# intel/pailliercryptolib

Hardware: AMD Instinct MI355X
Metric: 2048-bit modexps/sec (encrypt+decrypt) (higher is better)
Workload: dtype u64

## Files before the change

### pailliercryptolib_amd/csrc/hensel_ps_bal.hpp

```cpp
#ifndef PAILLIERCRYPTOLIB_AMD_CSRC_HENSEL_PS_BAL_HPP_
#define PAILLIERCRYPTOLIB_AMD_CSRC_HENSEL_PS_BAL_HPP_

#include "hensel_ps.hpp"

#ifndef PGPU_PSB_DOUBLED
#define PGPU_PSB_DOUBLED 1
#endif
#ifndef PGPU_PSB_KARATSUBA
#define PGPU_PSB_KARATSUBA 1
#endif

namespace pgpu {

template <int LB>
__device__ __forceinline__ int32_t psb_sext(uint32_t v) { return __builtin_amdgcn_sbfe((int)v, 0u, (unsigned)LB); }

__device__ __forceinline__ void psb_mac(int64_t& acc, int32_t x, int32_t y) { acc += (int64_t)x * y; }
__device__ __forceinline__ void psb_mac_pinned(int64_t& acc, int32_t x, int32_t y) {
  acc += (int64_t)x * y;
  asm volatile("" ::"v"(acc));
}

__device__ __forceinline__ void psb_mac_wrap(int64_t& acc, int32_t x, int32_t y) {
  acc = (int64_t)((uint64_t)acc + (uint64_t)((int64_t)x * y));
}

template <int K, int LB>
struct PsbFits {
  static constexpr bool value = 2 * (LB - 1) < 62 && LB + 6 < 62 &&
                                3 * (uint64_t)K * ((uint64_t)1 << (2 * (LB - 1))) + ((uint64_t)1 << (LB + 6)) < ((uint64_t)1 << 63);
};

template <int K, int LB, int NP, bool SYM, int QMODE, bool DBL = false, bool KARA = false>
__device__ __forceinline__ void psb_montmul(int32_t (&r)[K], const int32_t (&x1)[K], const int32_t (&y1)[K],
                                            const int32_t (&x2)[K], const int32_t (&y2)[K], const int32_t (&n)[K],
                                            uint32_t n0inv, int32_t (&qio)[K]) {
  static_assert(!(SYM && NP != 1), "a symmetric product is a single one");
  static_assert(SYM || !DBL, "the doubled operand belongs to the symmetric product");
  static_assert(!KARA || (NP == 1 && !SYM && K % 2 == 0), "the split serves the single product of two operands, in two halves");
  static_assert(PsbFits<K, LB>::value, "a column sums up to 3K products below 2^(2(LB-1)): must stay below 2^63");
  constexpr int H = K / 2;
  int32_t q[K];
  int64_t acc = 0;
  int32_t onev = 1;
  asm("" : "+v"(onev));
  int32_t dx[KARA ? H : 1], dy[KARA ? H : 1];
  uint64_t lo[KARA ? 2 * H - 1 : 1], hi[KARA ? 2 * H - 1 : 1];
  if constexpr (KARA) {
#pragma unroll
    for (int j = 0; j < H; ++j) {
      dx[j] = x1[j] - x1[H + j];
      dy[j] = y1[H + j] - y1[j];
    }
  }
  ps_static_for<2 * K>([&](auto colc) __attribute__((always_inline)) {
    constexpr int col = decltype(colc)::value;
    {
      constexpr int ilo = col < K ? 0 : col - K + 1;
      constexpr int ihi = col < K ? col : K;
      if constexpr (ihi > ilo) {
        ps_static_for<ihi - ilo>([&](auto ic) __attribute__((always_inline)) {
          constexpr int i = ilo + decltype(ic)::value;
          if constexpr (PGPU_PS_PIN == 2 || (PGPU_PS_PIN == 1 && SYM)) psb_mac_pinned(acc, q[i], n[col - i]);
          else psb_mac(acc, q[i], n[col - i]);
        });
      }
    }
    if constexpr (SYM) {
      constexpr int ilo = col < K ? 0 : col - K + 1;
      constexpr int ihi = (col + 1) / 2;
      if constexpr (DBL) {
        if constexpr (ihi > ilo) {
          ps_static_for<ihi - ilo>([&](auto ic) __attribute__((always_inline)) {
            constexpr int i = ilo + decltype(ic)::value;
            psb_mac(acc, x1[i], y1[col - i]);
          });
        }
        if constexpr (col % 2 == 0) psb_mac(acc, y1[col / 2], y1[col / 2]);
      } else {
        if constexpr (ihi > ilo) {
          int64_t cross = 0;
          ps_static_for<ihi - ilo>([&](auto ic) __attribute__((always_inline)) {
            constexpr int i = ilo + decltype(ic)::value;
            psb_mac(cross, x1[i], x1[col - i]);
          });
          acc = (int64_t)((uint64_t)acc + ((uint64_t)cross << 1));
        }
        if constexpr (col % 2 == 0) psb_mac(acc, x1[col / 2], x1[col / 2]);
      }
    } else if constexpr (KARA) {
      if constexpr (col <= 2 * H - 2) {
        constexpr int ilo = col < H ? 0 : col - H + 1;
        constexpr int ihi = col < H ? col + 1 : H;
        int64_t s = 0;
        ps_static_for<ihi - ilo>([&](auto ic) __attribute__((always_inline)) {
          constexpr int i = ilo + decltype(ic)::value;
          psb_mac_wrap(s, x1[i], y1[col - i]);
        });
        lo[col] = (uint64_t)s;
        acc = (int64_t)((uint64_t)acc + lo[col]);
      }
      if constexpr (col >= H && col <= 3 * H - 2) {
        constexpr int k = col - H;
        constexpr int ilo = k < H ? 0 : k - H + 1;
        constexpr int ihi = k < H ? k + 1 : H;
        int64_t s = 0;
        ps_static_for<ihi - ilo>([&](auto ic) __attribute__((always_inline)) {
          constexpr int i = ilo + decltype(ic)::value;
          psb_mac_wrap(s, x1[H + i], y1[H + k - i]);
        });
        hi[k] = (uint64_t)s;
        acc = (int64_t)((uint64_t)acc + (lo[k] + hi[k]));
        ps_static_for<ihi - ilo>([&](auto ic) __attribute__((always_inline)) {
          constexpr int i = ilo + decltype(ic)::value;
          psb_mac_wrap(acc, dx[i], dy[k - i]);
        });
      }
      if constexpr (col >= 2 * H && col <= 4 * H - 2) acc = (int64_t)((uint64_t)acc + hi[col - 2 * H]);
    } else {
      constexpr int ilo = col < K ? 0 : col - K + 1;
      constexpr int ihi = col < K ? col + 1 : K;
      ps_static_for<ihi - ilo>([&](auto ic) __attribute__((always_inline)) {
        constexpr int i = ilo + decltype(ic)::value;
        if constexpr (PGPU_PS_PIN == 2) {
          psb_mac_pinned(acc, x1[i], y1[col - i]);
          if constexpr (NP == 2) psb_mac_pinned(acc, x2[i], y2[col - i]);
        } else {
          psb_mac(acc, x1[i], y1[col - i]);
          if constexpr (NP == 2) psb_mac(acc, x2[i], y2[col - i]);
        }
      });
    }
    if constexpr (col < K) {
      if constexpr (QMODE == 2) psb_mac(acc, qio[col], onev);
      q[col] = psb_sext<LB>((uint32_t)acc * n0inv);
      psb_mac(acc, q[col], n[0]);
      acc >>= LB;
      if constexpr (QMODE == 1) qio[col] = q[col];
    } else {
      r[col - K] = psb_sext<LB>((uint32_t)acc);
      if constexpr (col + 1 < 2 * K) acc = (acc + ((int64_t)1 << (LB - 1))) >> LB;
    }
  });
}

template <int K>
__device__ __forceinline__ uint32_t (&psb_bits(int32_t (&v)[K]))[K] { return reinterpret_cast<uint32_t(&)[K]>(v); }
template <int K>
__device__ __forceinline__ const uint32_t (&psb_bits(const int32_t (&v)[K]))[K] { return reinterpret_cast<const uint32_t(&)[K]>(v); }

template <int K, int LB, bool DBL = (PGPU_PSB_DOUBLED != 0), bool KARA = (PGPU_PSB_KARATSUBA != 0)>
__device__ __forceinline__ void psb_pairsqr(int32_t (&a)[K], int32_t (&b)[K], const int32_t (&n)[K], uint32_t n0inv) {
  int32_t qd[K], t[K];
  if constexpr (DBL) {
    int32_t a2[K];
#pragma unroll
    for (int j = 0; j < K; ++j) a2[j] = a[j] * 2;
    psb_montmul<K, LB, 1, true, 1, true>(t, a2, a, a2, a, n, n0inv, qd);
    psb_montmul<K, LB, 1, false, 2, false, KARA>(b, a2, b, a2, b, n, n0inv, qd);
  } else {
    psb_montmul<K, LB, 1, true, 1>(t, a, a, a, a, n, n0inv, qd);
#pragma unroll
    for (int j = 0; j < K; ++j) b[j] *= 2;
    psb_montmul<K, LB, 1, false, 2>(b, a, b, a, b, n, n0inv, qd);
  }
#pragma unroll
  for (int j = 0; j < K; ++j) a[j] = t[j];
}

template <int K, int LB, bool KARA = (PGPU_PSB_KARATSUBA != 0)>
__device__ __forceinline__ void psb_pairmul(int32_t (&a)[K], int32_t (&b)[K], const int32_t (&c)[K], const int32_t (&d)[K],
                                            const int32_t (&n)[K], uint32_t n0inv, uint4* slot) {
  int32_t qd[K];
  {
    int32_t t[K];
    ps_park_store<K>(slot, psb_bits<K>(b));
    __builtin_amdgcn_sched_barrier(0);
    psb_montmul<K, LB, 1, false, 1, false, KARA>(t, a, c, a, c, n, n0inv, qd);
    __builtin_amdgcn_sched_barrier(0);
    ps_park_swap<K>(slot, psb_bits<K>(b), psb_bits<K>(t));
    __builtin_amdgcn_sched_barrier(0);
  }
  psb_montmul<K, LB, 2, false, 2>(b, a, d, b, c, n, n0inv, qd);
  __builtin_amdgcn_sched_barrier(0);
  ps_park_load<K>(psb_bits<K>(a), slot);
}

template <int K, int LB>
__device__ __forceinline__ void psb_mul(int32_t (&r)[K], const int32_t (&x)[K], const int32_t (&y)[K], const int32_t (&n)[K],
                                        uint32_t n0inv) {
  int32_t none[K];
  psb_montmul<K, LB, 1, false, 0>(r, x, y, x, y, n, n0inv, none);
}

template <int K, int LB>
__device__ __forceinline__ void psb_add(int32_t (&a)[K], const int32_t (&k)[K]) {
  int32_t c = 0;
#pragma unroll
  for (int j = 0; j < K; ++j) {
    const int32_t u = a[j] + k[j] + c;
    a[j] = j + 1 < K ? psb_sext<LB>((uint32_t)u) : u;
    c = (u + (1 << (LB - 1))) >> LB;
  }
}

template <int K, int LB, int NI>
__device__ __forceinline__ void psb_relimb(int32_t (&out)[K], const uint32_t (&in)[NI]) {
  static_assert(NI <= K, "the chunk must fit");
  uint32_t c = 0;
#pragma unroll
  for (int j = 0; j < K; ++j) {
    const uint32_t u = (j < NI ? in[j] : 0u) + c;
    out[j] = j + 1 < K ? psb_sext<LB>(u) : (int32_t)u;
    c = (u + (1u << (LB - 1))) >> LB;
  }
}

template <int K, int LB>
__device__ __forceinline__ int32_t psb_canon(uint32_t (&out)[K], const int32_t (&v)[K]) {
  int32_t c = 0;
#pragma unroll
  for (int j = 0; j < K; ++j) {
    const int32_t u = v[j] + c;
    out[j] = (uint32_t)u & PsLimb<LB>::mask;
    c = u >> LB;
  }
  return c;
}

template <int K, int LB>
__device__ __forceinline__ void psb_entry_from_pair_row(const HenselArgs& A, int side, size_t elem, const int32_t (&n)[K],
                                                        uint32_t n0inv, uint4* slot, int32_t (&a)[K], int32_t (&b)[K],
                                                        int32_t (&ma)[K], int32_t (&mb)[K]) {
  static_assert(LB == kLimbBits, "the row limbs are re-balanced, not re-cut");
  constexpr int NI = (K * LB - 2) / LB + 1;
#define HCTX(field) (side ? A.ctx[1].field : A.ctx[0].field)
  const uint32_t* row = A.ct_pair + elem * A.ct_pair_stride;
  int32_t acc_a[K], acc_b[K];
#pragma unroll
  for (int j = 0; j < K; ++j) acc_a[j] = acc_b[j] = 0;
#pragma unroll 1
  for (int i = 0; i < A.pchunks; ++i) {
    const int first = i * A.pchunk_limbs;
    uint32_t za[NI], zb[NI];
    int32_t cb[K], tb[K];
#pragma unroll
    for (int j = 0; j < NI; ++j) {
      const bool in = j < A.pchunk_limbs && first + j < A.pair_l2;
      za[j] = in ? row[first + j] : 0u;
      zb[j] = in ? row[A.pair_l2 + first + j] : 0u;
    }
#pragma unroll
    for (int j = 0; j < K; ++j) {
      b[j] = 0;
      cb[j] = (int32_t)HCTX(pcb)[(size_t)i * K + j];
      ma[j] = (int32_t)HCTX(pconv)[(size_t)i * 2 * K + j];
      mb[j] = (int32_t)HCTX(pconv)[(size_t)i * 2 * K + K + j];
    }
    int32_t zl[K];
    psb_relimb<K, LB, NI>(zl, zb);
    psb_mul<K, LB>(tb, zl, cb, n, n0inv);
    psb_relimb<K, LB, NI>(a, za);
    psb_pairmul<K, LB, false>(a, b, ma, mb, n, n0inv, slot);
    psb_add<K, LB>(b, tb);
    psb_add<K, LB>(acc_a, a);
    psb_add<K, LB>(acc_b, b);
  }
#pragma unroll
  for (int j = 0; j < K; ++j) {
    a[j] = ma[j] = acc_a[j];
    b[j] = mb[j] = acc_b[j];
  }
#undef HCTX
}

template <int K, int LB>
__device__ __forceinline__ void psb_exit_words(const HenselArgs& A, int side, size_t elem, bool live, uint4* slot,
                                               const int32_t (&n)[K], uint32_t n0inv, int32_t (&a)[K], int32_t (&b)[K],
                                               int32_t (&ma)[K], int32_t (&mb)[K]) {
  constexpr int W64 = (K * LB + 63) / 64;
#define HCTX(field) (side ? A.ctx[1].field : A.ctx[0].field)
#pragma unroll
  for (int j = 0; j < K; ++j) {
    ma[j] = (int32_t)HCTX(h)[j];
    mb[j] = 0;
  }
  psb_pairmul<K, LB, false>(a, b, ma, mb, n, n0inv, slot);
  uint32_t u0[K], u1[K];
  const int32_t neg_a = psb_canon<K, LB>(u0, a);
#pragma unroll
  for (int j = 0; j < K; ++j) ma[j] = a[j] - n[j];
  const int32_t below_p = psb_canon<K, LB>(u0, ma);
  const int32_t jflag = (below_p + 1) + neg_a;
#pragma unroll
  for (int j = 0; j < K; ++j) ma[j] = (j == 0 ? jflag : 0) - b[j];
  const int32_t neg_d = psb_canon<K, LB>(u0, ma);
#pragma unroll
  for (int j = 0; j < K; ++j) ma[j] += n[j];
  (void)psb_canon<K, LB>(u1, ma);
#pragma unroll
  for (int j = 0; j < K; ++j) u0[j] = neg_d ? u1[j] : u0[j];
  if (live) {
    uint64_t* out = A.out + (2 * elem + side) * A.out_stride;
    const int ow = A.out_words;
    ps_static_for<W64>([&](auto wc) __attribute__((always_inline)) {
      constexpr int ww = decltype(wc)::value;
      if (ww < ow) out[ww] = ps_word<K, LB, ww>(u0);
    });
    for (int ww = W64; ww < ow; ++ww) out[ww] = 0;
  }
#undef HCTX
}

template <int K, int LB, int MINW>
__global__ __launch_bounds__(kWGThreads, MINW) void hensel_decrypt_psb_kernel(HenselArgs A) {
  constexpr int K4 = (K + 3) / 4;
  raise_wave_priority();
  __shared__ uint4 park_[kWavesPerWG][K4][kWave];
  const int lane = threadIdx.x % kWave, wv = threadIdx.x / kWave;
  uint4* slot = &park_[wv][0][lane];
  const size_t wave_id = (size_t)blockIdx.x * kWavesPerWG + wv;
  const int side = __builtin_amdgcn_readfirstlane((int)(wave_id & 1));
  const size_t first_elem = (wave_id >> 1) * kWave;
  size_t elem = first_elem + lane;
  if (elem >= A.count) elem = A.count - 1;
#define HCTX(field) (side ? A.ctx[1].field : A.ctx[0].field)
  int32_t n[K], a[K], b[K], ma[K], mb[K];
#pragma unroll
  for (int j = 0; j < K; ++j) n[j] = (int32_t)ps_uniform(HCTX(nhat)[j]);
  const uint32_t n0inv = ps_uniform(HCTX(n0inv));
  const int w = A.window, tsize = 1 << w, half = tsize >> 1;
  const bool gather = A.ct_gather != 0;
  const bool odd = !gather && A.ps_odd_table != 0;
  uint4* tw = reinterpret_cast<uint4*>(A.table + wave_id * ps_table_words<K>(ps_table_entries(w, odd))) + lane;
  const uint64_t* ep = A.exp + (size_t)side * A.exp_stride;
  const int nwin = (A.exp_bits + w - 1) / w;
  auto digit = [&](int i) -> int {
    int bit = i * w;
    int word = bit >> 6, sh = bit & 63;
    uint64_t v = (word < A.exp_words) ? ep[word] >> sh : 0;
    if (sh + w > 64 && word + 1 < A.exp_words) v |= ep[word + 1] << (64 - sh);
    return (int)(v & (uint64_t)(tsize - 1));
  };

  psb_entry_from_pair_row<K, LB>(A, side, elem, n, n0inv, slot, a, b, ma, mb);
  ps_table_store<K>(tw, 1, psb_bits<K>(a), psb_bits<K>(b));
  {
    uint32_t oa[K], ob[K];
#pragma unroll
    for (int j = 0; j < K; ++j) {
      oa[j] = HCTX(one)[j];
      ob[j] = HCTX(one)[K + j];
    }
    ps_table_store<K>(tw, 0, oa, ob);
  }
#pragma unroll 1
  for (int k = odd ? 0 : 1; k < half && half > 1; ++k) {
    const bool sq = !odd || k == 0, mu = !odd || k > 0;
    ps_table_load<K>(psb_bits<K>(a), psb_bits<K>(b), tw, k > 1 ? k : 1, tsize, false);
    if (sq) {
      psb_pairsqr<K, LB>(a, b, n, n0inv);
      ps_table_store<K>(tw, odd ? half : 2 * k, psb_bits<K>(a), psb_bits<K>(b));
    }
    __builtin_amdgcn_sched_barrier(0);
    if (mu) {
      ps_table_load<K>(psb_bits<K>(ma), psb_bits<K>(mb), tw, odd ? half : 1, tsize, false);
      psb_pairmul<K, LB>(a, b, ma, mb, n, n0inv, slot);
      ps_table_store<K>(tw, odd ? k + 1 : 2 * k + 1, psb_bits<K>(a), psb_bits<K>(b));
    }
  }
#pragma unroll
  for (int j = 0; j < K; ++j) {
    a[j] = (int32_t)HCTX(one)[j];
    b[j] = (int32_t)HCTX(one)[K + j];
  }
  int win = nwin - 1;
  if (!odd && nwin > 0) {
    ps_table_load<K>(psb_bits<K>(a), psb_bits<K>(b), tw, digit(nwin - 1), tsize, gather);
    --win;
  }
#pragma unroll 1
  for (; win >= 0; --win) {
    const int wl = (odd && win == nwin - 1) ? A.exp_bits - win * w : w;
    int pos, idx;
    ps_window_place(digit(win), wl, odd, pos, idx);
#pragma unroll 1
    for (int i = 0; i <= wl; ++i) {
      if (i == pos) {
        ps_table_load<K>(psb_bits<K>(ma), psb_bits<K>(mb), tw, idx, tsize, gather);
        psb_pairmul<K, LB>(a, b, ma, mb, n, n0inv, slot);
      }
      if (i < wl) psb_pairsqr<K, LB>(a, b, n, n0inv);
    }
  }
  psb_exit_words<K, LB>(A, side, elem, first_elem + lane < A.count, slot, n, n0inv, a, b, ma, mb);
#undef HCTX
}

}

#endif
```

Baseline: 6.382 million.

## Fold Montgomery reduction's upper q·n product into Karatsuba chains

Extends the Karatsuba split used for the operand product so the reduction product q·n also uses a three-multiply split for its upper-half quadrant. It precomputes wave-uniform differences of the modulus halves (dn) and, once all q digits are known, computes q-half differences that ride on the existing lo/hi/middle chains. The aim is to drop part of the K² multiply-accumulates in each Karatsuba Montgomery multiply. In exchange it adds more live registers (dq, dn) and extra wrap-around accumulation, which could raise register pressure and cost occupancy.

```diff
diff --git a/pailliercryptolib_amd/csrc/hensel_ps_bal.hpp b/pailliercryptolib_amd/csrc/hensel_ps_bal.hpp
--- a/pailliercryptolib_amd/csrc/hensel_ps_bal.hpp
+++ b/pailliercryptolib_amd/csrc/hensel_ps_bal.hpp
@@ -9,6 +9,9 @@
 #ifndef PGPU_PSB_KARATSUBA
 #define PGPU_PSB_KARATSUBA 1
 #endif
+#ifndef PGPU_PSB_KARA_RED
+#define PGPU_PSB_KARA_RED 1
+#endif
 
 namespace pgpu {
 
@@ -31,13 +34,14 @@
                                 3 * (uint64_t)K * ((uint64_t)1 << (2 * (LB - 1))) + ((uint64_t)1 << (LB + 6)) < ((uint64_t)1 << 63);
 };
 
-template <int K, int LB, int NP, bool SYM, int QMODE, bool DBL = false, bool KARA = false>
+template <int K, int LB, int NP, bool SYM, int QMODE, bool DBL = false, bool KARA = false, bool KRED = false>
 __device__ __forceinline__ void psb_montmul(int32_t (&r)[K], const int32_t (&x1)[K], const int32_t (&y1)[K],
                                             const int32_t (&x2)[K], const int32_t (&y2)[K], const int32_t (&n)[K],
-                                            uint32_t n0inv, int32_t (&qio)[K]) {
+                                            const int32_t (&dn)[K / 2], uint32_t n0inv, int32_t (&qio)[K]) {
   static_assert(!(SYM && NP != 1), "a symmetric product is a single one");
   static_assert(SYM || !DBL, "the doubled operand belongs to the symmetric product");
   static_assert(!KARA || (NP == 1 && !SYM && K % 2 == 0), "the split serves the single product of two operands, in two halves");
+  static_assert(!KRED || KARA, "the folded reduction rides on the chains of the split product");
   static_assert(PsbFits<K, LB>::value, "a column sums up to 3K products below 2^(2(LB-1)): must stay below 2^63");
   constexpr int H = K / 2;
   int32_t q[K];
@@ -46,6 +50,7 @@
   asm("" : "+v"(onev));
   int32_t dx[KARA ? H : 1], dy[KARA ? H : 1];
   uint64_t lo[KARA ? 2 * H - 1 : 1], hi[KARA ? 2 * H - 1 : 1];
+  int32_t dq[KRED ? H : 1];
   if constexpr (KARA) {
 #pragma unroll
     for (int j = 0; j < H; ++j) {
@@ -55,7 +60,7 @@
   }
   ps_static_for<2 * K>([&](auto colc) __attribute__((always_inline)) {
     constexpr int col = decltype(colc)::value;
-    {
+    if constexpr (!KRED) {
       constexpr int ilo = col < K ? 0 : col - K + 1;
       constexpr int ihi = col < K ? col : K;
       if constexpr (ihi > ilo) {
@@ -63,6 +68,27 @@
           constexpr int i = ilo + decltype(ic)::value;
           if constexpr (PGPU_PS_PIN == 2 || (PGPU_PS_PIN == 1 && SYM)) psb_mac_pinned(acc, q[i], n[col - i]);
           else psb_mac(acc, q[i], n[col - i]);
+        });
+      }
+    } else {
+      if constexpr (col == K) {
+#pragma unroll
+        for (int j = 0; j < H; ++j) dq[j] = q[j] - q[H + j];
+      }
+      if constexpr (col > 0 && col < K) {
+        ps_static_for<col>([&](auto ic) __attribute__((always_inline)) {
+          constexpr int i = decltype(ic)::value;
+          if constexpr (!(col >= H && i < H && col - i < H)) {
+            if constexpr (PGPU_PS_PIN == 2 || (PGPU_PS_PIN == 1 && SYM)) psb_mac_pinned(acc, q[i], n[col - i]);
+            else psb_mac(acc, q[i], n[col - i]);
+          }
+        });
+      } else if constexpr (col >= K && col < K + H) {
+        constexpr int m = col - K;
+        ps_static_for<m + 1>([&](auto ic) __attribute__((always_inline)) {
+          constexpr int i = decltype(ic)::value;
+          if constexpr (PGPU_PS_PIN == 2 || (PGPU_PS_PIN == 1 && SYM)) psb_mac_pinned(acc, q[H + i], n[H + m - i]);
+          else psb_mac(acc, q[H + i], n[H + m - i]);
         });
       }
     }
@@ -97,6 +123,12 @@
           constexpr int i = ilo + decltype(ic)::value;
           psb_mac_wrap(s, x1[i], y1[col - i]);
         });
+        if constexpr (KRED && col >= H) {
+          ps_static_for<ihi - ilo>([&](auto ic) __attribute__((always_inline)) {
+            constexpr int i = ilo + decltype(ic)::value;
+            psb_mac_wrap(s, q[i], n[col - i]);
+          });
+        }
         lo[col] = (uint64_t)s;
         acc = (int64_t)((uint64_t)acc + lo[col]);
       }
@@ -109,12 +141,24 @@
           constexpr int i = ilo + decltype(ic)::value;
           psb_mac_wrap(s, x1[H + i], y1[H + k - i]);
         });
+        if constexpr (KRED && k >= H) {
+          ps_static_for<ihi - ilo>([&](auto ic) __attribute__((always_inline)) {
+            constexpr int i = ilo + decltype(ic)::value;
+            psb_mac_wrap(s, q[H + i], n[H + k - i]);
+          });
+        }
         hi[k] = (uint64_t)s;
         acc = (int64_t)((uint64_t)acc + (lo[k] + hi[k]));
         ps_static_for<ihi - ilo>([&](auto ic) __attribute__((always_inline)) {
           constexpr int i = ilo + decltype(ic)::value;
           psb_mac_wrap(acc, dx[i], dy[k - i]);
         });
+        if constexpr (KRED && k >= H) {
+          ps_static_for<ihi - ilo>([&](auto ic) __attribute__((always_inline)) {
+            constexpr int i = ilo + decltype(ic)::value;
+            psb_mac_wrap(acc, dq[i], dn[k - i]);
+          });
+        }
       }
       if constexpr (col >= 2 * H && col <= 4 * H - 2) acc = (int64_t)((uint64_t)acc + hi[col - 2 * H]);
     } else {
@@ -149,39 +193,42 @@
 template <int K>
 __device__ __forceinline__ const uint32_t (&psb_bits(const int32_t (&v)[K]))[K] { return reinterpret_cast<const uint32_t(&)[K]>(v); }
 
-template <int K, int LB, bool DBL = (PGPU_PSB_DOUBLED != 0), bool KARA = (PGPU_PSB_KARATSUBA != 0)>
-__device__ __forceinline__ void psb_pairsqr(int32_t (&a)[K], int32_t (&b)[K], const int32_t (&n)[K], uint32_t n0inv) {
+template <int K, int LB, bool DBL = (PGPU_PSB_DOUBLED != 0), bool KARA = (PGPU_PSB_KARATSUBA != 0),
+          bool KRED = (DBL && KARA && PGPU_PSB_KARA_RED != 0)>
+__device__ __forceinline__ void psb_pairsqr(int32_t (&a)[K], int32_t (&b)[K], const int32_t (&n)[K], const int32_t (&dn)[K / 2],
+                                            uint32_t n0inv) {
+  static_assert(!KRED || (DBL && KARA), "the folded reduction belongs to the doubled Karatsuba form");
   int32_t qd[K], t[K];
   if constexpr (DBL) {
     int32_t a2[K];
 #pragma unroll
     for (int j = 0; j < K; ++j) a2[j] = a[j] * 2;
-    psb_montmul<K, LB, 1, true, 1, true>(t, a2, a, a2, a, n, n0inv, qd);
-    psb_montmul<K, LB, 1, false, 2, false, KARA>(b, a2, b, a2, b, n, n0inv, qd);
+    psb_montmul<K, LB, 1, true, 1, true>(t, a2, a, a2, a, n, dn, n0inv, qd);
+    psb_montmul<K, LB, 1, false, 2, false, KARA, KRED>(b, a2, b, a2, b, n, dn, n0inv, qd);
   } else {
-    psb_montmul<K, LB, 1, true, 1>(t, a, a, a, a, n, n0inv, qd);
+    psb_montmul<K, LB, 1, true, 1>(t, a, a, a, a, n, dn, n0inv, qd);
 #pragma unroll
     for (int j = 0; j < K; ++j) b[j] *= 2;
-    psb_montmul<K, LB, 1, false, 2>(b, a, b, a, b, n, n0inv, qd);
+    psb_montmul<K, LB, 1, false, 2>(b, a, b, a, b, n, dn, n0inv, qd);
   }
 #pragma unroll
   for (int j = 0; j < K; ++j) a[j] = t[j];
 }
 
-template <int K, int LB, bool KARA = (PGPU_PSB_KARATSUBA != 0)>
+template <int K, int LB, bool KARA = (PGPU_PSB_KARATSUBA != 0), bool KRED = (KARA && PGPU_PSB_KARA_RED != 0)>
 __device__ __forceinline__ void psb_pairmul(int32_t (&a)[K], int32_t (&b)[K], const int32_t (&c)[K], const int32_t (&d)[K],
-                                            const int32_t (&n)[K], uint32_t n0inv, uint4* slot) {
+                                            const int32_t (&n)[K], const int32_t (&dn)[K / 2], uint32_t n0inv, uint4* slot) {
   int32_t qd[K];
   {
     int32_t t[K];
     ps_park_store<K>(slot, psb_bits<K>(b));
     __builtin_amdgcn_sched_barrier(0);
-    psb_montmul<K, LB, 1, false, 1, false, KARA>(t, a, c, a, c, n, n0inv, qd);
+    psb_montmul<K, LB, 1, false, 1, false, KARA, KRED>(t, a, c, a, c, n, dn, n0inv, qd);
     __builtin_amdgcn_sched_barrier(0);
     ps_park_swap<K>(slot, psb_bits<K>(b), psb_bits<K>(t));
     __builtin_amdgcn_sched_barrier(0);
   }
-  psb_montmul<K, LB, 2, false, 2>(b, a, d, b, c, n, n0inv, qd);
+  psb_montmul<K, LB, 2, false, 2>(b, a, d, b, c, n, dn, n0inv, qd);
   __builtin_amdgcn_sched_barrier(0);
   ps_park_load<K>(psb_bits<K>(a), slot);
 }
@@ -189,8 +236,8 @@
 template <int K, int LB>
 __device__ __forceinline__ void psb_mul(int32_t (&r)[K], const int32_t (&x)[K], const int32_t (&y)[K], const int32_t (&n)[K],
                                         uint32_t n0inv) {
-  int32_t none[K];
-  psb_montmul<K, LB, 1, false, 0>(r, x, y, x, y, n, n0inv, none);
+  int32_t none[K], nodn[K / 2] = {};
+  psb_montmul<K, LB, 1, false, 0>(r, x, y, x, y, n, nodn, n0inv, none);
 }
 
 template <int K, int LB>
@@ -236,7 +283,7 @@
   constexpr int NI = (K * LB - 2) / LB + 1;
 #define HCTX(field) (side ? A.ctx[1].field : A.ctx[0].field)
   const uint32_t* row = A.ct_pair + elem * A.ct_pair_stride;
-  int32_t acc_a[K], acc_b[K];
+  int32_t acc_a[K], acc_b[K], nodn[K / 2] = {};
 #pragma unroll
   for (int j = 0; j < K; ++j) acc_a[j] = acc_b[j] = 0;
 #pragma unroll 1
@@ -261,7 +308,7 @@
     psb_relimb<K, LB, NI>(zl, zb);
     psb_mul<K, LB>(tb, zl, cb, n, n0inv);
     psb_relimb<K, LB, NI>(a, za);
-    psb_pairmul<K, LB, false>(a, b, ma, mb, n, n0inv, slot);
+    psb_pairmul<K, LB, false>(a, b, ma, mb, n, nodn, n0inv, slot);
     psb_add<K, LB>(b, tb);
     psb_add<K, LB>(acc_a, a);
     psb_add<K, LB>(acc_b, b);
@@ -285,7 +332,8 @@
     ma[j] = (int32_t)HCTX(h)[j];
     mb[j] = 0;
   }
-  psb_pairmul<K, LB, false>(a, b, ma, mb, n, n0inv, slot);
+  int32_t nodn[K / 2] = {};
+  psb_pairmul<K, LB, false>(a, b, ma, mb, n, nodn, n0inv, slot);
   uint32_t u0[K], u1[K];
   const int32_t neg_a = psb_canon<K, LB>(u0, a);
 #pragma unroll
@@ -329,6 +377,9 @@
 #pragma unroll
   for (int j = 0; j < K; ++j) n[j] = (int32_t)ps_uniform(HCTX(nhat)[j]);
   const uint32_t n0inv = ps_uniform(HCTX(n0inv));
+  int32_t dn[K / 2];
+#pragma unroll
+  for (int j = 0; j < K / 2; ++j) dn[j] = PGPU_PSB_KARA_RED != 0 ? (int32_t)ps_uniform((uint32_t)(n[K / 2 + j] - n[j])) : 0;
   const int w = A.window, tsize = 1 << w, half = tsize >> 1;
   const bool gather = A.ct_gather != 0;
   const bool odd = !gather && A.ps_odd_table != 0;
@@ -359,13 +410,13 @@
     const bool sq = !odd || k == 0, mu = !odd || k > 0;
     ps_table_load<K>(psb_bits<K>(a), psb_bits<K>(b), tw, k > 1 ? k : 1, tsize, false);
     if (sq) {
-      psb_pairsqr<K, LB>(a, b, n, n0inv);
+      psb_pairsqr<K, LB>(a, b, n, dn, n0inv);
       ps_table_store<K>(tw, odd ? half : 2 * k, psb_bits<K>(a), psb_bits<K>(b));
     }
     __builtin_amdgcn_sched_barrier(0);
     if (mu) {
       ps_table_load<K>(psb_bits<K>(ma), psb_bits<K>(mb), tw, odd ? half : 1, tsize, false);
-      psb_pairmul<K, LB>(a, b, ma, mb, n, n0inv, slot);
+      psb_pairmul<K, LB>(a, b, ma, mb, n, dn, n0inv, slot);
       ps_table_store<K>(tw, odd ? k + 1 : 2 * k + 1, psb_bits<K>(a), psb_bits<K>(b));
     }
   }
@@ -388,9 +439,9 @@
     for (int i = 0; i <= wl; ++i) {
       if (i == pos) {
         ps_table_load<K>(psb_bits<K>(ma), psb_bits<K>(mb), tw, idx, tsize, gather);
-        psb_pairmul<K, LB>(a, b, ma, mb, n, n0inv, slot);
-      }
-      if (i < wl) psb_pairsqr<K, LB>(a, b, n, n0inv);
+        psb_pairmul<K, LB>(a, b, ma, mb, n, dn, n0inv, slot);
+      }
+      if (i < wl) psb_pairsqr<K, LB>(a, b, n, dn, n0inv);
     }
   }
   psb_exit_words<K, LB>(A, side, elem, first_elem + lane < A.count, slot, n, n0inv, a, b, ma, mb);
```

After: 6.517 million, median of 6. 1.02x the previous value.
